# jlvdb/yet_another_wizz

Measured on AMD Instinct MI355X. Metric: candidate pairs/s, higher is better.
Workload: dtype f64

## Files before the change

### yet_another_wizz_amd/csrc/yawhip_band32.inc

```
namespace {

constexpr int B32_WAVES_PLAIN = 7;
constexpr int B32_WAVES_BIG = 6;
constexpr int B32_WAVES_W = 5;
constexpr int B32_WAVES_W1 = 5;
constexpr int B32_WAVES_LT = 1;
constexpr int band32_min_waves(int R, int CAP, bool WEIGHTED, int NE, bool UNI) {
    if (NE == 2 && UNI) {
        if (WEIGHTED) return R == 1 ? B32_WAVES_W1 : B32_WAVES_W;
        return CAP >= B32_CAP_BIG ? B32_WAVES_BIG : B32_WAVES_PLAIN;
    }
    return NE == 2 && !WEIGHTED ? B32_WAVES_LT : 1;
}

template <int R, int CAP, bool WEIGHTED, int NE, bool MERGED, bool UNI>
__global__ __launch_bounds__(64, band32_min_waves(R, CAP, WEIGHTED, NE, UNI))
void YAW_B32_NAME(const DevTab *__restrict__ tabs, const Item *__restrict__ items, int n_bins,
                  const double *__restrict__ t, const float *__restrict__ thr32,
                  const double *__restrict__ rwin_k, const float *__restrict__ ucap,
                  unsigned flush_mask, int swap,
                  unsigned long long *__restrict__ out_counts,
                  double *__restrict__ partials,
                  unsigned long long *__restrict__ counters, unsigned long long seg_cap) {
    static_assert(NE >= 2 && NE <= 4, "edges per bin");
// ... 6 lines not shown
    constexpr int NC = NE == 2 ? 1 : NE;
    constexpr int NF = NE - 1;
    constexpr int TW = thr32_width(NE);
    constexpr bool LANE_THR = MERGED && !UNI;
    extern __shared__ __attribute__((aligned(16))) unsigned char lds_dyn[];
    const int nkb = MERGED ? n_bins : 1;
    const int nslots = nkb * NF;
    unsigned char *p = lds_dyn;
    constexpr bool SLOT_TRIP = NE == 2 && !WEIGHTED && R == 2 && !LANE_THR;
    constexpr bool DOWN = SLOT_TRIP && CH == 1;
    constexpr int LEAD = DOWN ? 4 : 0;
    constexpr unsigned COLB = (CAP + 4 + LEAD) * 4;
    float *const stage_lead = reinterpret_cast<float *>(p);
    float *stage = stage_lead + LEAD; p += (size_t)3 * COLB;
    double *sw = reinterpret_cast<double *>(p); if (WEIGHTED) p += (size_t)(CAP + 4) * 8;
    HistT *hist = reinterpret_cast<HistT *>(p); p += (size_t)nslots * sizeof(HistT);
    p = reinterpret_cast<unsigned char *>(((size_t)p + 15) & ~(size_t)15);
    float *sthr = reinterpret_cast<float *>(p);
    const int lane = threadIdx.x;
    const unsigned a_stage = (unsigned)(size_t)(lds_byte *)reinterpret_cast<unsigned char *>(stage);
    const unsigned a_sw = (unsigned)(size_t)(lds_byte *)reinterpret_cast<unsigned char *>(sw);
    const unsigned a_hist = (unsigned)(size_t)(lds_byte *)reinterpret_cast<unsigned char *>(hist);

    const TicketMap tmap = ticket_map(counters, seg_cap);
    const unsigned long long n_kept = tmap.n_kept;
    for (int e = lane; e < nslots; e += 64) hist[e] = HistT(0);
    if constexpr (DOWN) {
        if (a_stage != 4u * LEAD) __builtin_trap();
        if (lane < LEAD) { stage_lead[lane] = PAD_COORD32; stage_lead[COLB / 4 + lane] = PAD_COORD32; stage_lead[2 * (COLB / 4) + lane] = PAD_COORD32; }
    }
    if (LANE_THR)
        for (int e = lane; e < n_bins * TW; e += 64) sthr[e] = thr32[e];
    unsigned round_no = 0;
    for (unsigned long long v = blockIdx.x;; v += gridDim.x) {
        if ((v >> 3) >= tmap.per_xcd) break;
        const unsigned long long ticket = tmap.ticket(v);
        if (ticket >= n_kept) continue;
        const Item it = items[ticket];
        const int o = item_orient(it), islot = item_slot(it);
        const DevTab cl = tabs[swap ? o : 3 + o], cs = tabs[swap ? 3 + o : o];
        const int kfix = MERGED ? 0 : islot % n_bins;
        const float rwin = (float)(rwin_k[kfix] * 1.000001 + 4e-7);

        int win = 0;
        int64_t win_off = 0;
        int64_t cb[CH];
        int cn[CH], co[CH];
        int nch = 0;
        auto next_round = [&]() {
            nch = 0;
            int used = 0;
#pragma unroll
            for (int c = 0; c < CH; ++c) {
                cb[c] = 0; cn[c] = 0; co[c] = 0;
                if (win < it.nwin && nch == c) {
                    const int64_t wb = win == 0 ? it.b0[0] : (win == 1 ? it.b0[1] : it.b0[2]);
                    const int64_t rem = (int64_t)(win == 0 ? it.nb[0] : (win == 1 ? it.nb[1] : it.nb[2])) - win_off;
                    if (rem + 1 <= (int64_t)(CAP - used)) {
                        cb[c] = wb + win_off; cn[c] = (int)rem; co[c] = used;
                        used += ((int)rem + 1 + 3) & ~3;
                        ++win; win_off = 0; ++nch;
                    } else if (c == 0) {
                        cb[c] = wb + win_off; cn[c] = CAP - 4; co[c] = 0;
                        used = CAP;
                        win_off += CAP - 4; ++nch;
                    }
// ... 6 lines not shown
                if (c < nch) {
                    const gf32p gx = cs.qx + cb[c], gy = cs.qy + cb[c], gz = cs.qz + cb[c];
                    const unsigned a_c = a_stage + ((unsigned)co[c] << 2);
#pragma unroll
                    for (int k = 0; k < (CAP + 255) / 256; ++k) {
                        const unsigned e = (unsigned)(k * 256 + 4 * lane);
                        if (e < (unsigned)cn[c]) {
                            __builtin_amdgcn_global_load_lds(gx + e, lds_ptr(a_c + k * 1024), 16, 0, 0);
                            __builtin_amdgcn_global_load_lds(gy + e, lds_ptr(a_c + COLB + k * 1024), 16, 0, 0);
                            __builtin_amdgcn_global_load_lds(gz + e, lds_ptr(a_c + 2 * COLB + k * 1024), 16, 0, 0);
                        }
                    }
                    if (WEIGHTED && cs.w) {
#pragma unroll
                        for (int k = 0; k < (CAP + 127) / 128; ++k) {
                            const unsigned e = (unsigned)(k * 128 + 2 * lane);
                            if (e < (unsigned)cn[c])
                                __builtin_amdgcn_global_load_lds(cs.w + cb[c] + e, lds_ptr(a_sw + ((unsigned)co[c] << 3) + k * 1024), 16, 0, 0);
                        }
                    }
                }
            }
        };
        __syncthreads();
        next_round();
        issue_round();
        f32x2 ax2[R / 2 > 0 ? R / 2 : 1], ay2[R / 2 > 0 ? R / 2 : 1], az2[R / 2 > 0 ? R / 2 : 1];
        float ax[R], ay[R], az[R];
        int kb[R];
        double aw_own[R];
        int lane_obj = lane;
        int n_own = (int)it.na - lane * R;
        n_own = n_own < 0 ? 0 : (n_own > R ? R : n_own);
#pragma unroll
        for (int r = 0; r < R; ++r) {
            const bool have = r < n_own;
            const unsigned ic = have ? (unsigned)(lane * R + r) : 0u;
            ax[r] = have ? (cl.qx + it.a0)[ic] : PAD_COORD32;
            ay[r] = have ? (cl.qy + it.a0)[ic] : PAD_COORD32;
            az[r] = have ? (cl.qz + it.a0)[ic] : PAD_COORD32;
            kb[r] = MERGED ? (have ? (cl.k + it.a0)[ic] : 0) : 0;
            if constexpr (WEIGHTED) aw_own[r] = (cl.w && have) ? (cl.w + it.a0)[ic] : 1.0;
        }
        float th[R][TW];
        {
            const float *row = LANE_THR ? nullptr : thr32 + (size_t)kfix * TW;
#pragma unroll
            for (int r = 0; r < R; ++r)
#pragma unroll
                for (int q = 0; q < TW; ++q) th[r][q] = LANE_THR ? sthr[kb[r] * TW + q] : row[q];
        }
        float klo, khi;
        {
            const int last_r = n_own > 0 ? n_own - 1 : 0;
            float u_first = cl.axis == 0 ? ax[0] : (cl.axis == 1 ? ay[0] : az[0]), u_last = u_first;
#pragma unroll
            for (int r = 1; r < R; ++r)
                if (r == last_r) u_last = cl.axis == 0 ? ax[r] : (cl.axis == 1 ? ay[r] : az[r]);
            klo = u_first - rwin;
            khi = u_last + rwin;
            const float cap_c = ucap[2 * kfix], cap_s = ucap[2 * kfix + 1];
            if (cap_s > 0.0f) {
                klo = cap_lo32(u_first, cap_c, cap_s);
                khi = cap_hi32(u_last, cap_c, cap_s);
            }
        }
        if constexpr (R >= 2) {
#pragma unroll
            for (int h = 0; h < R / 2; ++h) {
                ax2[h] = f32x2{ax[2 * h], ax[2 * h + 1]}; ay2[h] = f32x2{ay[2 * h], ay[2 * h + 1]}; az2[h] = f32x2{az[2 * h], az[2 * h + 1]};
            }
        }
        f32x2 nc2[R / 2 > 0 ? R / 2 : 1];
#pragma unroll
        for (int h = 0; h < R / 2; ++h) nc2[h] = f32x2{-th[2 * h][0], -th[2 * h + 1][0]};
        unsigned int cnt[R][NC];
        double acc[R][NC];
#pragma unroll
        for (int r = 0; r < R; ++r)
#pragma unroll
            for (int c = 0; c < NC; ++c) { cnt[r][c] = 0u; acc[r][c] = 0.0; }
        unsigned int nev = 0;
        constexpr bool HALF = R == 1 && CH == 1;
        const double pair_mult = HALF && (it.pad_ & 1) ? 2.0 : 1.0;
        auto flush_lanes = [&]() {
#pragma unroll
            for (int r = 0; r < R; ++r) {
#pragma unroll
                for (int f = 0; f < NF; ++f) {
                    const unsigned cell = a_hist + (unsigned)((kb[r] * NF + f) * (int)sizeof(HistT));
                    if constexpr (WEIGHTED) {
                        const double vsum = NE == 2 ? acc[r][0] : acc[r][f + 1] - acc[r][f];
                        const double aw = aw_own[r];
                        if (vsum != 0.0)
                            (void)__hip_atomic_fetch_add((__attribute__((address_space(3))) double *)(size_t)cell, HALF ? aw * vsum * pair_mult : aw * vsum,
                                                         __ATOMIC_RELAXED, __HIP_MEMORY_SCOPE_WORKGROUP);
                    } else {
                        const unsigned int c = (NE == 2 ? cnt[r][0] : cnt[r][f + 1] - cnt[r][f]) << (HALF ? (it.pad_ & 1) : 0);
                        if (c)
                            (void)__hip_atomic_fetch_add((__attribute__((address_space(3))) unsigned int *)(size_t)cell, c,
                                                         __ATOMIC_RELAXED, __HIP_MEMORY_SCOPE_WORKGROUP);
                    }
                }
#pragma unroll
                for (int c = 0; c < NC; ++c) { cnt[r][c] = 0u; acc[r][c] = 0.0; }
            }
        };
        auto flush_counts = [&]() {
            flush_lanes();
            __syncthreads();
            for (int idx = lane; idx < nslots; idx += 64) {
                const unsigned int c = (unsigned int)hist[idx];
                hist[idx] = HistT(0);
                if (c) atomicAdd(&out_counts[(int64_t)islot * nslots + idx], (unsigned long long)c);
            }
        };

        const bool single_window = it.nwin == 1 && it.nb[0] + 1 <= CAP;
        for (;; ++round_no) {
            asm volatile("s_waitcnt vmcnt(0)" ::: "memory");
            __syncthreads();
            if (lane < nch) {
                int at = co[0] + cn[0];
                if constexpr (CH > 1) at = lane == 0 ? at : (lane == 1 ? co[1] + cn[1] : co[CH - 1] + cn[CH - 1]);
                stage[at] = PAD_COORD32; stage[COLB / 4 + at] = PAD_COORD32; stage[2 * (COLB / 4) + at] = PAD_COORD32;
                if (WEIGHTED) sw[at] = 0.0;
                if constexpr (PAIRS) {
                    stage[at + 1] = PAD_COORD32; stage[COLB / 4 + at + 1] = PAD_COORD32; stage[2 * (COLB / 4) + at + 1] = PAD_COORD32;
                    if (WEIGHTED) sw[at + 1] = 0.0;
                }
            }
            if (WEIGHTED && !cs.w) {
#pragma unroll
                for (int c = 0; c < CH; ++c)
                    if (c < nch)
                        for (int e = lane; e < cn[c]; e += 64) sw[co[c] + e] = 1.0;
            }
            __syncthreads();
            unsigned a_key[CH], a_sent[CH], ql[CH], qh[CH];
            int n_max = 1;
#pragma unroll
            for (int c = 0; c < CH; ++c) {
                a_key[c] = a_stage + COLB * (unsigned)cl.axis + ((unsigned)co[c] << 2);
                a_sent[c] = a_key[c] + ((unsigned)cn[c] << 2);
                ql[c] = qh[c] = a_key[c] - 4u;
                n_max = cn[c] > n_max ? cn[c] : n_max;
            }
            for (unsigned step = 4u << (31 - __builtin_clz(n_max)); step >= 4u; step >>= 1) {
#pragma unroll
                for (int c = 0; c < CH; ++c) {
                    if (c < nch) {
                        const unsigned pl = ql[c] + step, ph = qh[c] + step;
                        const float kl = *(const __attribute__((address_space(3))) float *)(size_t)(pl < a_sent[c] ? pl : a_sent[c]);
                        const float kh = *(const __attribute__((address_space(3))) float *)(size_t)(ph < a_sent[c] ? ph : a_sent[c]);
                        ql[c] = kl < klo ? pl : ql[c];
                        qh[c] = kh <= khi ? ph : qh[c];
                    }
                }
            }
#pragma unroll
            for (int c = 0; c < CH; ++c) {
            if (c < nch) {
            const int n = cn[c];
            int lo = (int)((ql[c] + 4u - a_key[c]) >> 2), hi = (int)((qh[c] + 4u - a_key[c]) >> 2);
            if (n_own == 0) lo = hi = n;
            if constexpr (R == 1 && CH == 1) {
                if (it.pad_ & 1) {
                    const int own = n_own > 0 ? (int)((long long)(cl.pos3 + it.a0)[lane] - (long long)cb[c]) + 1 : n;
                    lo = own > lo ? own : lo;
                    lo = lo > hi ? hi : lo;
                }
            }
            int len = hi - lo;
            int top = hi - 1;
            unsigned stride = PAIRS ? 8u : 4u;
            nev += (unsigned int)(len * n_own);
            if (single_window) {
                const unsigned long long act = __builtin_amdgcn_ballot_w64(len > 0);
                const int first = act ? __builtin_ctzll(act) : 0, span = act ? 64 - __builtin_clzll(act) - first : 64;
                if (span <= 32) {
                    const int sh = span <= 8 ? 3 : (span <= 16 ? 2 : 1);
                    const bool idle = (lane >> sh) >= span;
                    const int src = idle ? first : first + (lane >> sh);
                    const int part = lane & ((1 << sh) - 1);
                    if constexpr (R >= 2) {
#pragma unroll
                        for (int h = 0; h < R / 2; ++h) {
                            ax2[h] = f32x2{__shfl(ax2[h].x, src, 64), __shfl(ax2[h].y, src, 64)};
                            ay2[h] = f32x2{__shfl(ay2[h].x, src, 64), __shfl(ay2[h].y, src, 64)};
                            az2[h] = f32x2{__shfl(az2[h].x, src, 64), __shfl(az2[h].y, src, 64)};
                        }
                    }
#pragma unroll
                    for (int r = 0; r < R; ++r) {
                        if constexpr (R < 2) { ax[r] = __shfl(ax[r], src, 64); ay[r] = __shfl(ay[r], src, 64); az[r] = __shfl(az[r], src, 64); }
                        if constexpr (MERGED) kb[r] = __shfl(kb[r], src, 64);
                        if constexpr (WEIGHTED) aw_own[r] = __shfl(aw_own[r], src, 64);
// ... 192 lines not shown
                    }
                }
            } else {
                auto eval_entry = [&](const unsigned a16) {
                    unsigned long long unc_mask[NS];
                    float s32[NS];
                    double ewi[NS];
                    if (__builtin_expect(classify_entry(a16, unc_mask, s32, ewi) != 0ull, 0)) settle_entry(a16, unc_mask, s32, ewi);
                };
                for (int s = 0; s < steps; ++s) {
                    eval_entry(cur < last ? cur : last);
                    cur += stride;
                }
            }
            }
            }
            if (!WEIGHTED && (round_no & flush_mask) == flush_mask) flush_counts();
            if (win >= it.nwin) break;
            __syncthreads();
            next_round();
            issue_round();
        }
        ++round_no;
        if constexpr (WEIGHTED) {
            flush_lanes();
            __syncthreads();
            for (int idx = lane; idx < nslots; idx += 64) {
                partials[(int64_t)it.pot * nslots + idx] = (double)hist[idx];
                hist[idx] = HistT(0);
            }
        } else {
            flush_counts();
        }
        nev = wave_sum_lane63(nev);
        if (lane == 63 && nev) atomicAdd(&counters[BAND_ENTRY_CTR(ticket & (EVAL_SLOTS - 1))], (unsigned long long)nev);
    }
}

}

namespace yawhip_detail {

hipError_t YAW_B32_LAUNCH(const CountLaunch &L, bool wgt, int32_t *variant) {
    const std::pair<int, int> stage{L.R, L.cap};
    const std::pair<bool, bool> rows{L.merged, L.uni};
    const dim3 band_grid(L.band_grid), wave(64);
    return pick<Bool<false>, Bool<true>>(wgt, [&](auto w) {
        return pick<Int<4>, Int<3>, Int<2>>(L.n_edges, [&](auto ne) {
            return pick<Rows<true, false>, Rows<true, true>, Rows<false, true>>(rows, [&](auto r) {
                return pick<Stage<4, B32_CAP_BIG>, Stage<2, B32_CAP_BIG>, Stage<2, B32_CAP>, Stage<1, B32_CAP>>(stage, [&](auto s) {
                    using S = decltype(s);
                    using M = decltype(r);
                    *variant = variant_code(YAW_B32_CH == 1 ? VF_BAND32_ONE : VF_BAND32, S::R, S::CAP, w, ne, M::MERGED, M::UNI);
                    return launch(YAW_B32_NAME<S::R, S::CAP, w, ne, M::MERGED, M::UNI>, band_grid, wave, L.lds, L.stream, L.d_tabs,
                                  L.d_items, L.n_bins, L.d_t, L.d_thr32, L.d_rwin, L.d_ucap, L.flush_mask, L.swap ? 1 : 0,
                                  L.d_counts, L.d_partials, L.d_ctr, L.seg_cap);
                });
            });
        });
    });
}

}
```

### yet_another_wizz_amd/csrc/yawhip_count.hip

```cpp

#include <hip/hip_runtime.h>

#include <algorithm>
#include <chrono>
#include <cmath>
#include <cstdint>
#include <cstdio>
#include <cstring>
#include <functional>
#include <memory>
#include <new>
#include <numeric>
#include <utility>
#include <vector>

#include "yawhip_count_kernels.h"

using namespace yawhip_detail;

namespace {
inline DevTab make_tab(const double *x, const double *y, const double *z, const double *w, const int32_t *k, const int64_t *off,
                       const int64_t *vbase, const int64_t *slo, const int64_t *tiles, const TileRec *tile_rec, const RunGrid *grid,
                       int axis, const float *q = nullptr, int64_t q_stride = 0, const int32_t *idx = nullptr) {
    return DevTab{(gf64p)x, (gf64p)y, (gf64p)z, (gf64p)w, (gi32p)k, (gi64p)off, (gi64p)vbase, (gi64p)slo, (gi64p)tiles,
                  tile_rec, grid, (gf32p)q, (gf32p)(q ? q + q_stride : nullptr), (gf32p)(q ? q + 2 * q_stride : nullptr), (gi32p)idx,
                  (gi32p)nullptr, axis, 0};
}

inline int64_t seg_len(const yawhip_catalog *c, int patch, int k) {
    const int kk = c->nb == 1 ? 0 : k;
    const int64_t i = (int64_t)patch * c->nb + kk;
    return c->h_off[i + 1] - c->h_off[i];
}

int32_t merge_variant(int32_t a, int32_t b) { return a == 0 || a == b ? b : (b == 0 ? a : YAWHIP_VARIANT_MIXED); }

std::vector<float> build_thr32(const double *t, int n_bins, int n_edges) {
    auto down = [](double v) { float f = (float)v; if ((double)f > v) f = nextafterf(f, -INFINITY); return f; };
    auto up = [](double v) { float f = (float)v; if ((double)f < v) f = nextafterf(f, INFINITY); return f; };
    auto guard = [](double te) { return BAND32_GUARD_SQRT * std::sqrt(te) + 5e-7 * te + 1e-12; };
    const int tw = thr32_width(n_edges);
    std::vector<float> out((size_t)n_bins * tw, 0.f);
    for (int k = 0; k < n_bins; ++k) {
        const double *tk = t + (size_t)k * n_edges;
        float *row = &out[(size_t)k * tw];
        if (n_edges == 2) {
            const double g0 = guard(tk[0]), g1 = guard(tk[1]);
            const float c = (float)(0.5 * (tk[0] + tk[1]));
            const double cd = (double)c;
            const double fold = 4e-7 * cd;
            const double h_in = (std::min(cd - (tk[0] + g0), (tk[1] - g1) - cd) - fold) * (1.0 - 1e-6);
            const double h_out = (std::max(cd - (tk[0] - g0), (tk[1] + g1) - cd) + fold) * (1.0 + 1e-6);
            row[0] = c;
            row[1] = h_in > 0.0 ? down(h_in) : 0.f;
            row[2] = up(std::max(h_out, 0.0));
            row[3] = 0.f;
        } else {
            for (int e = 0; e < n_edges; ++e) {
                const double g = guard(tk[e]);
// ... 458 lines not shown
              ((P.run_weighted && n_items * P.slab * (int64_t)sizeof(double) > ctx->slab_budget) || n_items >= (1ll << 31));
    return YAWHIP_OK;
}

int Planner::tables() {
    std::vector<float> dthr((size_t)3 * n_bins);
    auto round_down = [](double v) { float f = (float)v; if ((double)f > v) f = nextafterf(f, -4.0f); return f; };
    for (int k = 0; k < n_bins; ++k) {
        const double thi = t[(size_t)k * n_edges + n_edges - 1];
        float thr32 = ctx->debug_no_hits ? 2.0f : round_down(1.0 - 0.5 * thi - FILTER_GUARD);
        dthr[(size_t)3 * k] = thr32;
        dthr[(size_t)3 * k + 1] = 0.f;
        dthr[(size_t)3 * k + 2] = 0.f;
    }
    if (P.merged) rwin[0] = P.rwin_max;
    const bool trim = ctx->band_trim && c1->unit_norm && c2->unit_norm;
    std::vector<float> ucap((size_t)2 * n_bins);
    for (int k = 0; k < n_bins; ++k) {
        const double th = sep_angle(rwin[(size_t)k]);
        ucap[(size_t)2 * k] = trim ? (float)std::cos(th) : 1.0f;
        ucap[(size_t)2 * k + 1] = trim ? (float)std::sin(th) : 0.0f;
    }
    if (trim) {
        P.cap_c = std::cos(sep_angle(P.rwin_max));
        P.cap_s = std::sin(sep_angle(P.rwin_max));
    }
    DevTab h_tabs[6];
    memset(h_tabs, 0, sizeof h_tabs);
    if (P.strip_items) {
        for (int o = 0; o < 3; ++o) {
            if (!L1[o]) continue;
            const StripLayout &a = *L1[o], &b = *L2[o];
            h_tabs[o] = make_tab(a.x, a.y, a.z, a.w, P.merged ? a.k : nullptr, a.off, a.d_vbase, a.d_slo, a.d_tiles[tile_idx],
                                 a.d_tile_rec[tile_idx], a.d_grid, o, a.q, a.q_stride);
            h_tabs[3 + o] = make_tab(b.x, b.y, b.z, b.w, nullptr, b.off, b.d_vbase, b.d_slo, b.d_tiles[tile_idx],
                                     b.d_tile_rec[tile_idx], b.d_grid, o, b.q, b.q_stride);
            if (P.triple) {
                const StripLayout &st = P.swap ? b : a;
                DevTab &tb = h_tabs[P.swap ? 3 + o : o];
                tb = make_tab(st.x, st.y, st.z, st.w3, nullptr, st.off3, st.d_vbase, st.d_slo, st.d_tiles[tile_idx],
                              st.d_tile_rec[tile_idx], st.d_grid3, o, st.q3, st.q3_stride, st.idx3);
                if (half_ok) h_tabs[3 + o].pos3 = (gi32p)(const int32_t *)b.pos3;
            }
        }
    } else {
        h_tabs[0] = make_tab(c1->x, c1->y, c1->z, c1->w, nullptr, c1->off, nullptr, nullptr, nullptr, nullptr, nullptr, c1->axis);
        h_tabs[3] = make_tab(c2->x, c2->y, c2->z, c2->w, nullptr, c2->off, nullptr, nullptr, nullptr, nullptr, nullptr, c2->axis);
    }
    static_assert(sizeof(JobRec) == 8 * sizeof(int32_t), "JobRec is 32 bytes");
    const std::vector<float> thr32 = P.band32 ? build_thr32(t, n_bins, n_edges) : (P.band_fine ? fine32 : std::vector<float>());
    std::vector<int64_t> cprefix;
    if (P.run_weighted) {
        cprefix.assign((size_t)P.n_pslots + 1, 0);
        for (int64_t sl = 0; sl < P.n_pslots; ++sl)
            cprefix[(size_t)sl + 1] = cprefix[(size_t)sl] + (prefix[(size_t)sl + 1] - prefix[(size_t)sl] + REDUCE_CHUNK - 1) / REDUCE_CHUNK;
    }
    P.n_chunks = cprefix.empty() ? 0 : cprefix.back();
    const void *src[9] = {P.strip_items ? (const void *)job_recs.data() : (const void *)jobs, prefix.data(), t, dthr.data(),
                          rwin.data(), ucap.data(), thr32.data(), h_tabs, cprefix.data()};
    const size_t bytes[9] = {P.strip_items ? sizeof(JobRec) * (size_t)P.n_sjobs : sizeof(int32_t) * 2 * (size_t)n_jobs,
                             sizeof(int64_t) * ((size_t)P.n_pslots + 1), sizeof(double) * n_bins * n_edges, sizeof(float) * 3 * n_bins,
                             sizeof(double) * n_bins, sizeof(float) * 2 * n_bins, sizeof(float) * thr32.size(), sizeof h_tabs,
                             sizeof(int64_t) * cprefix.size()};
    size_t off[9], off_in = 0;
    for (int i = 0; i < 9; ++i) { off[i] = off_in; off_in = align16(off_in + bytes[i]); }
    std::vector<unsigned char> image(off_in, 0);
    for (int i = 0; i < 9; ++i)
        if (bytes[i]) memcpy(image.data() + off[i], src[i], bytes[i]);
    HIP_TRY(P.d_in.alloc(std::max<size_t>(off_in, 16)));
// ... 448 lines not shown
```

### yet_another_wizz_amd/csrc/yawhip_count_device.h

```cpp
#ifndef YAWHIP_COUNT_DEVICE_H
#define YAWHIP_COUNT_DEVICE_H
#include <hip/hip_runtime.h>

#include <algorithm>
#include <cstdint>
#include <type_traits>
#include <utility>

#include "yawhip_count_kernels.h"

using namespace yawhip_detail;

namespace {
constexpr double PAD_COORD = 4.0;

struct alignas(16) ObjF {
    float x, y, z, pad;
};

__device__ __forceinline__ double cap_lo64(double u, double c, double s) {
    const double ul = fmax(u - 1e-9, -1.0);
    return ul <= -c + 1e-12 ? -1.0 - 2e-9 : fma(ul, c, -sqrt(fmax(fma(-ul, ul, 1.0), 0.0)) * s) - 2e-9;
}
__device__ __forceinline__ double cap_hi64(double u, double c, double s) {
    const double uh = fmin(u + 1e-9, 1.0);
    return uh >= c - 1e-12 ? 1.0 + 2e-9 : fma(uh, c, sqrt(fmax(fma(-uh, uh, 1.0), 0.0)) * s) + 2e-9;
}
constexpr float CAP32_SHIFT = 1e-7f, CAP32_CLIP = 1.2e-7f, CAP32_MARGIN = 8e-7f;
__device__ __forceinline__ float cap_lo32(float u, float c, float s) {
    const float ul = fmaxf(u - CAP32_SHIFT, -1.0f);
    return ul <= -c + CAP32_CLIP ? -1.0f - CAP32_MARGIN : fmaf(ul, c, -sqrtf(fmaxf(fmaf(-ul, ul, 1.0f), 0.0f)) * s) - CAP32_MARGIN;
}
__device__ __forceinline__ float cap_hi32(float u, float c, float s) {
    const float uh = fminf(u + CAP32_SHIFT, 1.0f);
    return uh >= c - CAP32_CLIP ? 1.0f + CAP32_MARGIN : fmaf(uh, c, sqrtf(fmaxf(fmaf(-uh, uh, 1.0f), 0.0f)) * s) + CAP32_MARGIN;
}

constexpr int SLOT_MASK = 0x3fffffff;
__host__ __device__ inline int item_slot(const Item &it) { return it.slot & SLOT_MASK; }
__host__ __device__ inline int item_orient(const Item &it) { return (int)((unsigned)it.slot >> 30); }

typedef float f32x2 __attribute__((ext_vector_type(2)));
typedef float f32x4 __attribute__((ext_vector_type(4)));

__device__ __forceinline__ void stamp_start(unsigned long long *__restrict__ counters, int word) {
    if (blockIdx.x == 0 && threadIdx.x == 0) counters[word] = wall_clock64();
}

typedef __attribute__((address_space(3))) unsigned char lds_byte;
__device__ __forceinline__ __attribute__((address_space(3))) void *lds_ptr(unsigned addr) { return (__attribute__((address_space(3))) void *)(size_t)addr; }
__device__ __forceinline__ double lds_f64(unsigned addr) { return *(const __attribute__((address_space(3))) double *)(size_t)addr; }
__device__ __forceinline__ int lds_i32(unsigned addr) { return *(const __attribute__((address_space(3))) int *)(size_t)addr; }

__device__ __forceinline__ int wave_max_nonneg(int v) {
    v = max(v, __builtin_amdgcn_update_dpp(0, v, 0x111, 0xf, 0xf, false));
    v = max(v, __builtin_amdgcn_update_dpp(0, v, 0x112, 0xf, 0xf, false));
    v = max(v, __builtin_amdgcn_update_dpp(0, v, 0x114, 0xf, 0xf, false));
    v = max(v, __builtin_amdgcn_update_dpp(0, v, 0x118, 0xf, 0xf, false));
    v = max(v, __builtin_amdgcn_update_dpp(0, v, 0x142, 0xa, 0xf, false));
    v = max(v, __builtin_amdgcn_update_dpp(0, v, 0x143, 0xc, 0xf, false));
    return __builtin_amdgcn_readlane(v, 63);
}

__device__ __forceinline__ unsigned int wave_sum_lane63(unsigned int v) {
    v += (unsigned int)__builtin_amdgcn_update_dpp(0, (int)v, 0x111, 0xf, 0xf, false);
    v += (unsigned int)__builtin_amdgcn_update_dpp(0, (int)v, 0x112, 0xf, 0xf, false);
    v += (unsigned int)__builtin_amdgcn_update_dpp(0, (int)v, 0x114, 0xf, 0xf, false);
    v += (unsigned int)__builtin_amdgcn_update_dpp(0, (int)v, 0x118, 0xf, 0xf, false);
// ... 112 lines not shown
```

### yet_another_wizz_amd/csrc/yawhip_ingest.hip

```cpp

#include <hip/hip_runtime.h>

#include <algorithm>
#include <atomic>
#include <climits>
#include <cmath>
#include <cstdint>
#include <cstring>
#include <new>
#include <vector>

#include "yawhip_internal.h"

using namespace yawhip_detail;

namespace {

__global__ __launch_bounds__(256) void k_assign_patches(int64_t n, const double *__restrict__ x, const double *__restrict__ y,
                                                       const double *__restrict__ z, int n_centers,
                                                       const double *__restrict__ centers, int32_t *__restrict__ out) {
    extern __shared__ __attribute__((aligned(16))) unsigned char lds_raw[];
    double *c = reinterpret_cast<double *>(lds_raw);
    for (int e = threadIdx.x; e < 3 * n_centers; e += blockDim.x) c[e] = centers[e];
    __syncthreads();
// ... 54 lines not shown
}

__global__ __launch_bounds__(256) void k_segment_weight_sums(const double *__restrict__ w, const int64_t *__restrict__ off,
                                                            double *__restrict__ out) {
    __shared__ double part[256];
    const int64_t lo = off[blockIdx.x], hi = off[blockIdx.x + 1];
    double acc = 0.0;
    for (int64_t i = lo + threadIdx.x; i < hi; i += 256) acc += w[i];
    part[threadIdx.x] = acc;
    __syncthreads();
    for (int half = 128; half > 0; half >>= 1) {
        if ((int)threadIdx.x < half) part[threadIdx.x] += part[threadIdx.x + half];
        __syncthreads();
    }
    if (threadIdx.x == 0) out[blockIdx.x] = part[0];
}

__device__ __forceinline__ int segment_of(const int64_t *__restrict__ off, int n_seg, int64_t i) {
    int lo = 0, hi = n_seg;
    while (hi - lo > 1) {
        const int mid = (lo + hi) >> 1;
        if (off[mid] <= i) lo = mid; else hi = mid;
    }
    return lo;
}

__global__ void k_gather_bins(int64_t n, const uint32_t *__restrict__ perm, const int64_t *__restrict__ off, int64_t n_seg,
                              int n_bins, int32_t *__restrict__ bins) {
    const int64_t i = (int64_t)blockIdx.x * blockDim.x + threadIdx.x;
    if (i < n) bins[i] = segment_of(off, (int)n_seg, (int64_t)perm[i]) % n_bins;
}

__global__ void k_make_q(int64_t n, const double *__restrict__ x, const double *__restrict__ y, const double *__restrict__ z,
                         int64_t stride, float *__restrict__ q) {
    const int64_t i = (int64_t)blockIdx.x * blockDim.x + threadIdx.x;
    if (i >= n) return;
    q[i] = (float)x[i];
    q[stride + i] = (float)y[i];
    q[2 * stride + i] = (float)z[i];
}

__global__ void k_same_bin_neighbours(int64_t n, const int32_t *__restrict__ bins, unsigned long long *__restrict__ out) {
    const int64_t i = (int64_t)blockIdx.x * blockDim.x + threadIdx.x;
    const bool same = i + 1 < n && bins[i] == bins[i + 1];
    const unsigned long long m = __builtin_amdgcn_ballot_w64(same);
    if ((threadIdx.x & 63) == 0 && m) atomicAdd(out, (unsigned long long)__popcll(m));
}

__global__ void k_strip_index(int64_t n, const double *__restrict__ v, const double *__restrict__ u, const double *__restrict__ w,
                              double width, int lat, const int64_t *__restrict__ poff, int n_patches, int32_t *__restrict__ gidx,
                              int32_t *__restrict__ lohi) {
    const int64_t i = (int64_t)blockIdx.x * blockDim.x + threadIdx.x;
    const bool ok = i < n;
    int32_t g = 0;
    int p = -1;
    if (ok) {
        const double vi = v[i];
        if (width > 0.0)
            g = lat ? (int32_t)floor((atan2(vi, hypot(u[i], w[i])) + 1.5707963267948966) / width) : (int32_t)floor((vi + 1.0) / width);
        gidx[i] = g;
        p = segment_of(poff, n_patches, i);
    }
    const int p0 = __builtin_amdgcn_readfirstlane(p);
    if (__builtin_amdgcn_ballot_w64(p != p0) == 0ull) {
        if (p0 < 0) return;
        int32_t lo = g, hi = g;
        for (int off = 32; off > 0; off >>= 1) {
            lo = min(lo, __shfl_xor(lo, off, 64));
            hi = max(hi, __shfl_xor(hi, off, 64));
        }
        if ((threadIdx.x & 63) == 0) {
            atomicMin(&lohi[2 * p0], lo);
// ... 202 lines not shown
                       key_of(c->x, c->y, c->z, (saxis + 1) % 3), key_of(c->x, c->y, c->z, (saxis + 2) % 3), width, c->strip_grid && !seg ? 1 : 0, poff,
                       n_groups, gidx, lohi);
    e = hipMemcpyAsync(h_lohi.data(), lohi, (size_t)2 * n_groups * sizeof(int32_t), hipMemcpyDeviceToHost, ctx->stream);
    if (e == hipSuccess) e = hipStreamSynchronize(ctx->stream);
    if (e != hipSuccess) return bail(e, "strip index");
    std::vector<int64_t> vbase((size_t)n_groups + 1, 0), slo((size_t)n_groups, 0);
    for (int g = 0; g < n_groups; ++g) {
        const bool any = h_poff[(size_t)g + 1] > h_poff[(size_t)g];
        slo[(size_t)g] = any ? h_lohi[(size_t)2 * g] : 0;
        vbase[(size_t)g + 1] = vbase[(size_t)g] + (any ? (int64_t)h_lohi[(size_t)2 * g + 1] - h_lohi[(size_t)2 * g] + 1 : 0);
    }
    const int64_t n_runs = vbase[(size_t)n_groups];
    if (n_runs >= (1ll << 31)) return bail(hipErrorInvalidValue, "too many strip runs");
    int run_bits = 1;
    while ((1ll << run_bits) < n_runs) ++run_bits;
    e = L.d_vbase.alloc((size_t)(n_groups + 1));
    if (e == hipSuccess) e = L.d_slo.alloc((size_t)std::max(n_groups, 1));
    if (e == hipSuccess)
        e = hipMemcpyAsync(L.d_vbase, vbase.data(), (size_t)(n_groups + 1) * sizeof(int64_t), hipMemcpyHostToDevice, ctx->stream);
    if (e == hipSuccess)
        e = hipMemcpyAsync(L.d_slo, slo.data(), (size_t)n_groups * sizeof(int64_t), hipMemcpyHostToDevice, ctx->stream);
    if (e == hipSuccess) e = yawsort::sort_segments(ctx->sort_ws, ctx->stream, n, key_of(c->x, c->y, c->z, o), poff, n_groups, perm);
    if (e != hipSuccess) return bail(e, "group sort");
    hipLaunchKernelGGL(k_run_of, dim3(ngrid), dim3(256), 0, ctx->stream, n, perm, gidx, poff, n_groups, L.d_vbase, L.d_slo, run);
    e = yawsort::sort_runs(ctx->sort_ws, ctx->stream, n, run, perm, run_bits, perm2, run_sorted);
    if (e != hipSuccess) return bail(e, "run sort");
    e = L.x.alloc(n1, 16);
    if (e == hipSuccess) e = L.y.alloc(n1, 16);
    if (e == hipSuccess) e = L.z.alloc(n1, 16);
    if (e == hipSuccess && c->w) e = L.w.alloc(n1, 16);
    if (e == hipSuccess && want_bins) e = L.k.alloc(n1, 16);
    L.q_stride = (int64_t)((n1 + 3) & ~(size_t)3) + 8;
    if (e == hipSuccess) e = L.q.alloc((size_t)3 * L.q_stride);
    if (e == hipSuccess) e = L.off.alloc((size_t)(n_runs + 1));
    if (e == hipSuccess) e = L.d_grid.alloc((size_t)(n_runs + 1));
    if (e == hipSuccess) e = hipMemsetAsync(L.d_grid, 0, (size_t)(n_runs + 1) * sizeof(RunGrid), ctx->stream);
    if (e != hipSuccess) return bail(e, "strip layout");
    hipLaunchKernelGGL(k_gather_columns, dim3(ngrid), dim3(256), 0, ctx->stream, n, perm2, c->x, c->y, c->z, c->w, L.x, L.y, L.z, L.w);
    if (want_bins)
        hipLaunchKernelGGL(k_gather_bins, dim3(ngrid), dim3(256), 0, ctx->stream, n, perm2, c->off, nseg, c->nb, L.k);
    hipLaunchKernelGGL(k_make_q, dim3(ngrid), dim3(256), 0, ctx->stream, n, L.x, L.y, L.z, L.q_stride, L.q);
    hipLaunchKernelGGL(k_run_offsets, dim3((unsigned)((n_runs + 1 + 255) / 256)), dim3(256), 0, ctx->stream, run_sorted, n, n_runs,
                       L.off);
    if (n_runs > 0)
        hipLaunchKernelGGL(k_run_grid<double>, dim3((unsigned)((n_runs * (RUN_GRID + 1) + 255) / 256)), dim3(256), 0, ctx->stream, n_runs,
                           L.off, o == 0 ? L.x : (o == 1 ? L.y : L.z), L.d_grid);
    std::vector<int64_t> voff((size_t)n_runs + 1);
    e = hipMemcpyAsync(voff.data(), L.off, (size_t)(n_runs + 1) * sizeof(int64_t), hipMemcpyDeviceToHost, ctx->stream);
    unsigned long long h_same = 0;
    if (want_bins && n > 1) {
        unsigned long long *d_same = reinterpret_cast<unsigned long long *>(static_cast<uint32_t *>(run));
        if (e == hipSuccess) e = hipMemsetAsync(d_same, 0, sizeof(unsigned long long), ctx->stream);
        if (e == hipSuccess) {
            hipLaunchKernelGGL(k_same_bin_neighbours, dim3(ngrid), dim3(256), 0, ctx->stream, n, L.k, d_same);
            e = hipMemcpyAsync(&h_same, d_same, sizeof(unsigned long long), hipMemcpyDeviceToHost, ctx->stream);
        }
    }
    if (e == hipSuccess) e = hipStreamSynchronize(ctx->stream);
    if (e != hipSuccess) return bail(e, "run offsets");
    L.same_bin = n > 1 ? (double)h_same / (double)(n - 1) : 0.0;
    for (int64_t r = 0; r < n_runs; ++r)
        if (voff[(size_t)r + 1] - voff[(size_t)r] >= (1ll << 32)) return bail(hipErrorInvalidValue, "a strip run of 2^32 objects or more");
    for (int ri = 0; ri < 3; ++ri) {
        const int64_t tile = (int64_t)MWG << ri;
        L.h_tiles[ri].assign((size_t)n_runs + 1, 0);
        for (int64_t r = 0; r < n_runs; ++r)
            L.h_tiles[ri][(size_t)r + 1] = L.h_tiles[ri][(size_t)r] + (voff[(size_t)r + 1] - voff[(size_t)r] + tile - 1) / tile;
        {
            const int64_t n_tiles = L.h_tiles[ri][(size_t)n_runs];
            std::vector<TileRec> tile_rec((size_t)std::max<int64_t>(n_tiles, 1), TileRec{0, 0, 0, 0.0, 0.0});
            for (int64_t r = 0; r < n_runs; ++r)
                for (int64_t tl = L.h_tiles[ri][(size_t)r]; tl < L.h_tiles[ri][(size_t)r + 1]; ++tl) {
                    const int64_t a0 = voff[(size_t)r] + (tl - L.h_tiles[ri][(size_t)r]) * tile;
                    tile_rec[(size_t)tl] = TileRec{a0, (int32_t)std::min<int64_t>(tile, voff[(size_t)r + 1] - a0), (int32_t)r, 0.0, 0.0};
// ... 268 lines not shown
    return upload_catalogs(ctx, n, x, y, z, w, kappa ? kappa : &none, n_patches, n_bins_or_1, offsets, sort_axis, out_n, out_k);
}

int yawhip_catalog_segment_sums(const yawhip_catalog *cat, double *sums) {
    if (!cat || !sums) return fail(YAWHIP_ERR_INVALID, "yawhip_catalog_segment_sums: NULL argument");
    const int64_t nseg = (int64_t)cat->n_patches * cat->nb;
    if (!cat->w) {
        for (int64_t s = 0; s < nseg; ++s) sums[s] = (double)(cat->h_off[(size_t)s + 1] - cat->h_off[(size_t)s]);
        return YAWHIP_OK;
    }
    yawhip_ctx *ctx = cat->ctx;
    HIP_TRY(hipSetDevice(ctx->device));
    DevPtr<double> d_out;
    hipError_t e = d_out.alloc((size_t)nseg);
    if (e != hipSuccess) return fail(YAWHIP_ERR_OOM, "segment sums: %s", hipGetErrorString(e));
    hipLaunchKernelGGL(k_segment_weight_sums, dim3((unsigned)nseg), dim3(256), 0, ctx->stream, cat->w, cat->off, d_out);
    e = hipGetLastError();
    if (e == hipSuccess) e = hipMemcpyAsync(sums, d_out, (size_t)nseg * sizeof(double), hipMemcpyDeviceToHost, ctx->stream);
    if (e == hipSuccess) e = hipStreamSynchronize(ctx->stream);
    if (e != hipSuccess) return fail(YAWHIP_ERR_HIP, "segment sums failed: %s", hipGetErrorString(e));
    return YAWHIP_OK;
}

int yawhip_catalog_free(yawhip_catalog *c) {
    if (!c) return YAWHIP_OK;
    for (yawhip_catalog *rep : c->replicas) (void)yawhip_catalog_free(rep);
    c->replicas.clear();
    if (c->ctx) (void)hipSetDevice(c->ctx->device);
    if (c->ctx) {
        if (c->ctx->stream) (void)hipStreamSynchronize(c->ctx->stream);
        drop_plans(c->ctx, c);
    }
    delete c;
    return YAWHIP_OK;
}

int yawhip_catalog_device_bytes(const yawhip_catalog *cat, int64_t *bytes) {
    if (!cat || !bytes) return fail(YAWHIP_ERR_INVALID, "yawhip_catalog_device_bytes: NULL argument");
    *bytes = cat->device_bytes;
    return YAWHIP_OK;
}

int yawhip_assign_patches(yawhip_ctx *ctx, int64_t n, const double *x, const double *y, const double *z, int32_t n_centers,
                          const double *centers_xyz, int32_t *patch_out) {
    if (!ctx) return fail(YAWHIP_ERR_INVALID, "yawhip_assign_patches: ctx is NULL");
    if (n < 0 || n_centers <= 0 || !centers_xyz || (n > 0 && (!x || !y || !z || !patch_out)))
        return fail(YAWHIP_ERR_INVALID, "yawhip_assign_patches: bad sizes or NULL arrays");
    if ((size_t)n_centers * 3 * sizeof(double) > (size_t)ctx->lds_limit)
        return fail(YAWHIP_ERR_INVALID, "too many centres (%d) for the LDS table", n_centers);
    if (n == 0) return YAWHIP_OK;
    HIP_TRY(hipSetDevice(ctx->device));
    DevPtr<double> dx, dc;
    DevPtr<int32_t> dout;
    hipError_t e = dx.alloc((size_t)3 * n);
    if (e == hipSuccess) e = dc.alloc((size_t)3 * n_centers);
    if (e == hipSuccess) e = dout.alloc((size_t)n);
    if (e == hipSuccess) e = hipMemcpyAsync(dx, x, (size_t)n * sizeof(double), hipMemcpyHostToDevice, ctx->stream);
    if (e == hipSuccess) e = hipMemcpyAsync(dx + n, y, (size_t)n * sizeof(double), hipMemcpyHostToDevice, ctx->stream);
    if (e == hipSuccess) e = hipMemcpyAsync(dx + 2 * n, z, (size_t)n * sizeof(double), hipMemcpyHostToDevice, ctx->stream);
    if (e == hipSuccess)
        e = hipMemcpyAsync(dc, centers_xyz, (size_t)3 * n_centers * sizeof(double), hipMemcpyHostToDevice, ctx->stream);
    if (e == hipSuccess) {
        const size_t lds = (size_t)3 * n_centers * sizeof(double);
        if (lds > 64 * 1024)
            e = hipFuncSetAttribute(reinterpret_cast<const void *>(k_assign_patches), hipFuncAttributeMaxDynamicSharedMemorySize, (int)lds);
        if (e == hipSuccess) {
// ... 13 lines not shown
```

### yet_another_wizz_amd/csrc/yawhip_internal.h

```cpp
#ifndef YAWHIP_INTERNAL_H
#define YAWHIP_INTERNAL_H
#include <hip/hip_runtime.h>

#include <chrono>
#include <cstddef>
#include <cstdint>
#include <cstdio>
#include <cstdlib>
#include <cstring>
#include <functional>
#include <string>
#include <utility>
#include <vector>

#include "yawhip.h"
#include "yawhip_devmem.h"
#include "yawhip_healpix.h"
#include "yawhip_sort.h"

#pragma GCC visibility push(hidden)

namespace yawhip_detail {
struct Trace {
    bool on = getenv("YAWHIP_TRACE") != nullptr;
// ... 31 lines not shown
#define HIP_TRY(expr)                                                                              \
    do {                                                                                           \
        hipError_t e_ = (expr);                                                                    \
        if (e_ != hipSuccess)                                                                      \
            return fail(e_ == hipErrorOutOfMemory ? YAWHIP_ERR_OOM : YAWHIP_ERR_HIP, "%s failed: %s (%s:%d)", \
                        #expr, hipGetErrorString(e_), __FILE__, __LINE__);                         \
    } while (0)

struct CatView {
    const double *x, *y, *z, *w;
    const int64_t *off;
    int nb;
    const double *key;
    int axis;
};

constexpr int MAX_WIN = 3;
struct alignas(16) Item {
    int64_t a0;
    int32_t na;
    int32_t slot;
    int32_t pot;
    int32_t nwin;
    int64_t b0[MAX_WIN];
    int32_t nb[MAX_WIN];
    int32_t pad_;
};
static_assert(sizeof(Item) == 64, "Item layout");

typedef const __attribute__((address_space(1))) double *gf64p;
typedef const __attribute__((address_space(1))) int32_t *gi32p;
typedef const __attribute__((address_space(1))) int64_t *gi64p;
typedef const __attribute__((address_space(1))) float *gf32p;
struct DevTab {
    gf64p x, y, z, w;
    gi32p k;
    gi64p off;
    gi64p vbase, slo, tiles;
    const struct TileRec *tile_rec;
    const struct RunGrid *grid;
    gf32p qx, qy, qz;
    gi32p idx;
    gi32p pos3;
    int32_t axis;
    int32_t pad_;
};
__device__ __forceinline__ gf64p tab_key(const DevTab &t) { return t.axis == 0 ? t.x : (t.axis == 1 ? t.y : t.z); }

struct alignas(16) TileRec {
    int64_t a0;
    int32_t na;
    int32_t run;
    double klo, khi;
};
static_assert(sizeof(TileRec) == 32, "TileRec is read as two 16-byte words");
struct JobRec {
    int64_t t_lo;
    int64_t k_off;
    int64_t vbase1;
    int32_t n_strips1;
    int32_t o;
};
constexpr int RUN_GRID = 64;
struct alignas(16) RunGrid {
    int64_t b0;
    double first, last;
    double inv;
    uint32_t n;
    uint32_t g[RUN_GRID + 1];
};
static_assert(sizeof(RunGrid) == 304 && offsetof(RunGrid, n) == 32, "RunGrid: a 36-byte head in front of g[]");
constexpr int64_t RUN_GRID_ACCOUNTED = 8 + 4 * (RUN_GRID + 2), TILE_REC_ACCOUNTED = 16;
__device__ __forceinline__ int run_cell(double key, double first, double inv) {
    const double f = (key - first) * inv;
// ... 87 lines not shown
    const double *t = nullptr;
    std::vector<int32_t> own_jobs;
    std::vector<double> own_t;

    CallKey() = default;
    CallKey(const yawhip_ctx *ctx, const CountArgs &a, bool want_counts, bool want_sums, bool for_work,
            int32_t n_dev = 0);
    CallKey(CallKey &&) = default;
    CallKey &operator=(CallKey &&) = default;
    CallKey(const CallKey &) = delete;
    CallKey &operator=(const CallKey &) = delete;

    void keep() {
        own_jobs.assign(jobs, jobs + 2 * (size_t)n_jobs);
        own_t.assign(t, t + (size_t)n_bins * n_edges);
        jobs = own_jobs.data();
        t = own_t.data();
    }
    bool operator==(const CallKey &o) const {
        return hash == o.hash && c1_uid == o.c1_uid && c2_uid == o.c2_uid && opt_gen == o.opt_gen && n_jobs == o.n_jobs &&
               n_bins == o.n_bins && n_edges == o.n_edges && kernel == o.kernel && n_dev == o.n_dev && want_counts == o.want_counts &&
               want_sums == o.want_sums && for_work == o.for_work &&
               memcmp(jobs, o.jobs, sizeof(int32_t) * 2 * (size_t)n_jobs) == 0 &&
               memcmp(t, o.t, sizeof(double) * (size_t)n_bins * n_edges) == 0;
    }
};

struct StripLayout {
    bool built = false;
    DevPtr<double> x, y, z, w;
    DevPtr<int32_t> k;
    DevPtr<float> q;
    int64_t q_stride = 0;
    DevPtr<int64_t> off;
    std::vector<int64_t> h_off;
    std::vector<int64_t> h_vbase;
    std::vector<int64_t> h_slo;
    std::vector<int64_t> h_tiles[3];
    DevPtr<int64_t> d_vbase, d_slo, d_tiles[3];
    DevPtr<TileRec> d_tile_rec[3];
    DevPtr<RunGrid> d_grid;
    bool triples = false;
    DevPtr<float> q3;
    int64_t q3_stride = 0;
    DevPtr<double> w3;
    DevPtr<int32_t> idx3;
    DevPtr<int32_t> pos3;
    DevPtr<int64_t> off3;
    DevPtr<RunGrid> d_grid3;
    int64_t n_groups = 0;
    int64_t device_bytes = 0;
    double obj_run = 0.0;
    double same_bin = 0.0;
    void release_triples() {
        q3.release(); w3.release(); idx3.release(); pos3.release(); off3.release(); d_grid3.release();
        triples = false;
    }
    void release() { *this = StripLayout{}; }
};

}

struct yawhip_ctx : yawhip_detail::CallBufs {
    int device = 0;
    hipStream_t stream = nullptr;
    int tile_r = 0;
// ... 123 lines not shown
```

Before: 35060000 billion.

## Pack per-object coords and bin into 16-byte records; rework band search and entry counting

Adds an interleaved float4 image (x,y,z,bin) per strip layout so each lane loads its owned objects with a single 16-byte load instead of four separate strided loads. The binary search over staged keys changes from a clamped power-of-two step search to a halving-count search with a final fix-up compare, which drops the per-step sentinel clamp. Entry-counter atomics are batched across tickets and only flushed when a lane counter nears overflow, and the cap bound computations use the raw hardware sqrt. The cost is extra device memory and ingest work for the new image, plus a debug entry point to check it.

```diff
diff --git a/yet_another_wizz_amd/csrc/yawhip_band32.inc b/yet_another_wizz_amd/csrc/yawhip_band32.inc
--- a/yet_another_wizz_amd/csrc/yawhip_band32.inc
+++ b/yet_another_wizz_amd/csrc/yawhip_band32.inc
@@ -62,6 +62,12 @@
     if (LANE_THR)
         for (int e = lane; e < n_bins * TW; e += 64) sthr[e] = thr32[e];
     unsigned round_no = 0;
+    unsigned int nev = 0;
+    auto send_entries = [&](unsigned int lane_sum) {
+        const unsigned int lo16 = wave_sum_lane63(lane_sum & 0xffffu), hi16 = wave_sum_lane63(lane_sum >> 16);
+        const unsigned long long sum = (unsigned long long)lo16 + ((unsigned long long)hi16 << 16);
+        if (lane == 63 && sum) atomicAdd(&counters[BAND_ENTRY_CTR(blockIdx.x & (EVAL_SLOTS - 1))], sum);
+    };
     for (unsigned long long v = blockIdx.x;; v += gridDim.x) {
         if ((v >> 3) >= tmap.per_xcd) break;
         const unsigned long long ticket = tmap.ticket(v);
@@ -134,14 +140,20 @@
         int lane_obj = lane;
         int n_own = (int)it.na - lane * R;
         n_own = n_own < 0 ? 0 : (n_own > R ? R : n_own);
+        lane_words rec[R];
+        {
+            const glanep lane_q = cl.q4 + it.a0 + lane * R;
+#pragma unroll
+            for (int r = 0; r < R; ++r) rec[r] = lane_q[r];
+        }
 #pragma unroll
         for (int r = 0; r < R; ++r) {
             const bool have = r < n_own;
             const unsigned ic = have ? (unsigned)(lane * R + r) : 0u;
-            ax[r] = have ? (cl.qx + it.a0)[ic] : PAD_COORD32;
-            ay[r] = have ? (cl.qy + it.a0)[ic] : PAD_COORD32;
-            az[r] = have ? (cl.qz + it.a0)[ic] : PAD_COORD32;
-            kb[r] = MERGED ? (have ? (cl.k + it.a0)[ic] : 0) : 0;
+            ax[r] = have ? rec[r].x : PAD_COORD32;
+            ay[r] = have ? rec[r].y : PAD_COORD32;
+            az[r] = have ? rec[r].z : PAD_COORD32;
+            kb[r] = MERGED ? (have ? __float_as_int(rec[r].w) : 0) : 0;
             if constexpr (WEIGHTED) aw_own[r] = (cl.w && have) ? (cl.w + it.a0)[ic] : 1.0;
         }
         float th[R][TW];
@@ -182,7 +194,6 @@
         for (int r = 0; r < R; ++r)
 #pragma unroll
             for (int c = 0; c < NC; ++c) { cnt[r][c] = 0u; acc[r][c] = 0.0; }
-        unsigned int nev = 0;
         constexpr bool HALF = R == 1 && CH == 1;
         const double pair_mult = HALF && (it.pad_ & 1) ? 2.0 : 1.0;
         auto flush_lanes = [&]() {
@@ -239,24 +250,26 @@
                         for (int e = lane; e < cn[c]; e += 64) sw[co[c] + e] = 1.0;
             }
             __syncthreads();
-            unsigned a_key[CH], a_sent[CH], ql[CH], qh[CH];
-            int n_max = 1;
+            unsigned a_key[CH], ql[CH], qh[CH];
+            int left[CH], left_max = 0;
 #pragma unroll
             for (int c = 0; c < CH; ++c) {
                 a_key[c] = a_stage + COLB * (unsigned)cl.axis + ((unsigned)co[c] << 2);
-                a_sent[c] = a_key[c] + ((unsigned)cn[c] << 2);
                 ql[c] = qh[c] = a_key[c] - 4u;
-                n_max = cn[c] > n_max ? cn[c] : n_max;
-            }
-            for (unsigned step = 4u << (31 - __builtin_clz(n_max)); step >= 4u; step >>= 1) {
+                left[c] = cn[c];
+                left_max = cn[c] > left_max ? cn[c] : left_max;
+            }
+            for (; left_max > 1; left_max -= left_max >> 1) {
 #pragma unroll
                 for (int c = 0; c < CH; ++c) {
-                    if (c < nch) {
-                        const unsigned pl = ql[c] + step, ph = qh[c] + step;
-                        const float kl = *(const __attribute__((address_space(3))) float *)(size_t)(pl < a_sent[c] ? pl : a_sent[c]);
-                        const float kh = *(const __attribute__((address_space(3))) float *)(size_t)(ph < a_sent[c] ? ph : a_sent[c]);
+                    if (c < nch && (CH == 1 || left[c] > 1)) {
+                        const unsigned half4 = (unsigned)(left[c] >> 1) << 2;
+                        const unsigned pl = ql[c] + half4, ph = qh[c] + half4;
+                        const float kl = *(const __attribute__((address_space(3))) float *)(size_t)pl;
+                        const float kh = *(const __attribute__((address_space(3))) float *)(size_t)ph;
                         ql[c] = kl < klo ? pl : ql[c];
                         qh[c] = kh <= khi ? ph : qh[c];
+                        left[c] -= left[c] >> 1;
                     }
                 }
             }
@@ -265,6 +278,8 @@
             if (c < nch) {
             const int n = cn[c];
             int lo = (int)((ql[c] + 4u - a_key[c]) >> 2), hi = (int)((qh[c] + 4u - a_key[c]) >> 2);
+            lo += *(const __attribute__((address_space(3))) float *)(size_t)(ql[c] + 4u) < klo ? 1 : 0;
+            hi += *(const __attribute__((address_space(3))) float *)(size_t)(qh[c] + 4u) <= khi ? 1 : 0;
             if (n_own == 0) lo = hi = n;
             if constexpr (R == 1 && CH == 1) {
                 if (it.pad_ & 1) {
@@ -523,9 +538,9 @@
         } else {
             flush_counts();
         }
-        nev = wave_sum_lane63(nev);
-        if (lane == 63 && nev) atomicAdd(&counters[BAND_ENTRY_CTR(ticket & (EVAL_SLOTS - 1))], (unsigned long long)nev);
+        if (__builtin_amdgcn_ballot_w64((int)nev < 0)) { send_entries(nev); nev = 0; }
     }
+    send_entries(nev);
 }
 
 }
diff --git a/yet_another_wizz_amd/csrc/yawhip_count.hip b/yet_another_wizz_amd/csrc/yawhip_count.hip
--- a/yet_another_wizz_amd/csrc/yawhip_count.hip
+++ b/yet_another_wizz_amd/csrc/yawhip_count.hip
@@ -21,10 +21,11 @@
 namespace {
 inline DevTab make_tab(const double *x, const double *y, const double *z, const double *w, const int32_t *k, const int64_t *off,
                        const int64_t *vbase, const int64_t *slo, const int64_t *tiles, const TileRec *tile_rec, const RunGrid *grid,
-                       int axis, const float *q = nullptr, int64_t q_stride = 0, const int32_t *idx = nullptr) {
+                       int axis, const float *q = nullptr, int64_t q_stride = 0, const int32_t *idx = nullptr,
+                       const LaneObj *q4 = nullptr) {
     return DevTab{(gf64p)x, (gf64p)y, (gf64p)z, (gf64p)w, (gi32p)k, (gi64p)off, (gi64p)vbase, (gi64p)slo, (gi64p)tiles,
-                  tile_rec, grid, (gf32p)q, (gf32p)(q ? q + q_stride : nullptr), (gf32p)(q ? q + 2 * q_stride : nullptr), (gi32p)idx,
-                  (gi32p)nullptr, axis, 0};
+                  tile_rec, grid, (gf32p)q, (gf32p)(q ? q + q_stride : nullptr), (gf32p)(q ? q + 2 * q_stride : nullptr), (glanep)q4,
+                  (gi32p)idx, (gi32p)nullptr, axis, 0};
 }
 
 inline int64_t seg_len(const yawhip_catalog *c, int patch, int k) {
@@ -549,9 +550,9 @@
             if (!L1[o]) continue;
             const StripLayout &a = *L1[o], &b = *L2[o];
             h_tabs[o] = make_tab(a.x, a.y, a.z, a.w, P.merged ? a.k : nullptr, a.off, a.d_vbase, a.d_slo, a.d_tiles[tile_idx],
-                                 a.d_tile_rec[tile_idx], a.d_grid, o, a.q, a.q_stride);
+                                 a.d_tile_rec[tile_idx], a.d_grid, o, a.q, a.q_stride, nullptr, a.q4);
             h_tabs[3 + o] = make_tab(b.x, b.y, b.z, b.w, nullptr, b.off, b.d_vbase, b.d_slo, b.d_tiles[tile_idx],
-                                     b.d_tile_rec[tile_idx], b.d_grid, o, b.q, b.q_stride);
+                                     b.d_tile_rec[tile_idx], b.d_grid, o, b.q, b.q_stride, nullptr, b.q4);
             if (P.triple) {
                 const StripLayout &st = P.swap ? b : a;
                 DevTab &tb = h_tabs[P.swap ? 3 + o : o];
diff --git a/yet_another_wizz_amd/csrc/yawhip_count_device.h b/yet_another_wizz_amd/csrc/yawhip_count_device.h
--- a/yet_another_wizz_amd/csrc/yawhip_count_device.h
+++ b/yet_another_wizz_amd/csrc/yawhip_count_device.h
@@ -27,13 +27,17 @@
     return uh >= c - 1e-12 ? 1.0 + 2e-9 : fma(uh, c, sqrt(fmax(fma(-uh, uh, 1.0), 0.0)) * s) + 2e-9;
 }
 constexpr float CAP32_SHIFT = 1e-7f, CAP32_CLIP = 1.2e-7f, CAP32_MARGIN = 8e-7f;
+__device__ __forceinline__ float cap32_clipped(float bound) {
+    asm volatile("" : "+v"(bound));
+    return bound;
+}
 __device__ __forceinline__ float cap_lo32(float u, float c, float s) {
-    const float ul = fmaxf(u - CAP32_SHIFT, -1.0f);
-    return ul <= -c + CAP32_CLIP ? -1.0f - CAP32_MARGIN : fmaf(ul, c, -sqrtf(fmaxf(fmaf(-ul, ul, 1.0f), 0.0f)) * s) - CAP32_MARGIN;
+    const float ul = fmaxf(u - CAP32_SHIFT, -1.0f), clipped = cap32_clipped(-1.0f - CAP32_MARGIN);
+    return ul <= -c + CAP32_CLIP ? clipped : fmaf(ul, c, -__builtin_amdgcn_sqrtf(fmaxf(fmaf(-ul, ul, 1.0f), 0.0f)) * s) - CAP32_MARGIN;
 }
 __device__ __forceinline__ float cap_hi32(float u, float c, float s) {
-    const float uh = fminf(u + CAP32_SHIFT, 1.0f);
-    return uh >= c - CAP32_CLIP ? 1.0f + CAP32_MARGIN : fmaf(uh, c, sqrtf(fmaxf(fmaf(-uh, uh, 1.0f), 0.0f)) * s) + CAP32_MARGIN;
+    const float uh = fminf(u + CAP32_SHIFT, 1.0f), clipped = cap32_clipped(1.0f + CAP32_MARGIN);
+    return uh >= c - CAP32_CLIP ? clipped : fmaf(uh, c, __builtin_amdgcn_sqrtf(fmaxf(fmaf(-uh, uh, 1.0f), 0.0f)) * s) + CAP32_MARGIN;
 }
 
 constexpr int SLOT_MASK = 0x3fffffff;
diff --git a/yet_another_wizz_amd/csrc/yawhip_ingest.hip b/yet_another_wizz_amd/csrc/yawhip_ingest.hip
--- a/yet_another_wizz_amd/csrc/yawhip_ingest.hip
+++ b/yet_another_wizz_amd/csrc/yawhip_ingest.hip
@@ -110,12 +110,18 @@
 }
 
 __global__ void k_make_q(int64_t n, const double *__restrict__ x, const double *__restrict__ y, const double *__restrict__ z,
-                         int64_t stride, float *__restrict__ q) {
-    const int64_t i = (int64_t)blockIdx.x * blockDim.x + threadIdx.x;
-    if (i >= n) return;
-    q[i] = (float)x[i];
-    q[stride + i] = (float)y[i];
-    q[2 * stride + i] = (float)z[i];
+                         const int32_t *__restrict__ bins, int64_t stride, float *__restrict__ q, LaneObj *__restrict__ q4) {
+    const int64_t i = (int64_t)blockIdx.x * blockDim.x + threadIdx.x;
+    if (i >= n + LANE_IMAGE_PAD) return;
+    if (i >= n) {
+        q4[i] = LaneObj{0.0f, 0.0f, 0.0f, 0};
+        return;
+    }
+    const float fx = (float)x[i], fy = (float)y[i], fz = (float)z[i];
+    q[i] = fx;
+    q[stride + i] = fy;
+    q[2 * stride + i] = fz;
+    q4[i] = LaneObj{fx, fy, fz, bins ? bins[i] : 0};
 }
 
 __global__ void k_same_bin_neighbours(int64_t n, const int32_t *__restrict__ bins, unsigned long long *__restrict__ out) {
@@ -384,6 +390,7 @@
     if (e == hipSuccess && want_bins) e = L.k.alloc(n1, 16);
     L.q_stride = (int64_t)((n1 + 3) & ~(size_t)3) + 8;
     if (e == hipSuccess) e = L.q.alloc((size_t)3 * L.q_stride);
+    if (e == hipSuccess) e = L.q4.alloc((size_t)(n + LANE_IMAGE_PAD));
     if (e == hipSuccess) e = L.off.alloc((size_t)(n_runs + 1));
     if (e == hipSuccess) e = L.d_grid.alloc((size_t)(n_runs + 1));
     if (e == hipSuccess) e = hipMemsetAsync(L.d_grid, 0, (size_t)(n_runs + 1) * sizeof(RunGrid), ctx->stream);
@@ -391,7 +398,8 @@
     hipLaunchKernelGGL(k_gather_columns, dim3(ngrid), dim3(256), 0, ctx->stream, n, perm2, c->x, c->y, c->z, c->w, L.x, L.y, L.z, L.w);
     if (want_bins)
         hipLaunchKernelGGL(k_gather_bins, dim3(ngrid), dim3(256), 0, ctx->stream, n, perm2, c->off, nseg, c->nb, L.k);
-    hipLaunchKernelGGL(k_make_q, dim3(ngrid), dim3(256), 0, ctx->stream, n, L.x, L.y, L.z, L.q_stride, L.q);
+    hipLaunchKernelGGL(k_make_q, dim3((unsigned)((n + LANE_IMAGE_PAD + 255) / 256)), dim3(256), 0, ctx->stream, n, L.x, L.y, L.z,
+                       want_bins ? (const int32_t *)L.k : nullptr, L.q_stride, L.q, L.q4);
     hipLaunchKernelGGL(k_run_offsets, dim3((unsigned)((n_runs + 1 + 255) / 256)), dim3(256), 0, ctx->stream, run_sorted, n, n_runs,
                        L.off);
     if (n_runs > 0)
@@ -726,6 +734,30 @@
         drop_plans(c->ctx, c);
     }
     delete c;
+    return YAWHIP_OK;
+}
+
+int yawhip_debug_lane_image(yawhip_ctx *ctx, yawhip_catalog *cat, int32_t o, int32_t seg, int64_t *n_checked, int64_t *n_differing) {
+    if (!ctx || !cat || !n_checked || !n_differing || o < 0 || o > 2) return fail(YAWHIP_ERR_INVALID, "yawhip_debug_lane_image: bad argument");
+    if (cat->strip_width <= 0.0 || (seg && cat->nb <= 1)) return fail(YAWHIP_ERR_INVALID, "yawhip_debug_lane_image: no such layout");
+    if (const int rc = build_strip_layout(ctx, cat, o, seg != 0)) return rc;
+    const StripLayout &L = seg ? cat->seg[o] : cat->strips[o];
+    const int64_t n = cat->n;
+    std::vector<LaneObj> rec((size_t)(n + LANE_IMAGE_PAD));
+    std::vector<float> q((size_t)3 * L.q_stride);
+    std::vector<int32_t> bins((size_t)n, 0);
+    HIP_TRY(hipSetDevice(ctx->device));
+    HIP_TRY(hipMemcpy(rec.data(), L.q4, rec.size() * sizeof(LaneObj), hipMemcpyDeviceToHost));
+    HIP_TRY(hipMemcpy(q.data(), L.q, q.size() * sizeof(float), hipMemcpyDeviceToHost));
+    if (L.k && n > 0) HIP_TRY(hipMemcpy(bins.data(), L.k, (size_t)n * sizeof(int32_t), hipMemcpyDeviceToHost));
+    int64_t bad = 0;
+    for (int64_t i = 0; i < n + LANE_IMAGE_PAD; ++i) {
+        const LaneObj want = i < n ? LaneObj{q[(size_t)i], q[(size_t)(L.q_stride + i)], q[(size_t)(2 * L.q_stride + i)], bins[(size_t)i]}
+                                   : LaneObj{0.0f, 0.0f, 0.0f, 0};
+        bad += memcmp(&rec[(size_t)i], &want, sizeof(LaneObj)) != 0;
+    }
+    *n_checked = n;
+    *n_differing = bad;
     return YAWHIP_OK;
 }
 
diff --git a/yet_another_wizz_amd/csrc/yawhip_internal.h b/yet_another_wizz_amd/csrc/yawhip_internal.h
--- a/yet_another_wizz_amd/csrc/yawhip_internal.h
+++ b/yet_another_wizz_amd/csrc/yawhip_internal.h
@@ -87,6 +87,14 @@
 typedef const __attribute__((address_space(1))) int32_t *gi32p;
 typedef const __attribute__((address_space(1))) int64_t *gi64p;
 typedef const __attribute__((address_space(1))) float *gf32p;
+struct alignas(16) LaneObj {
+    float x, y, z;
+    int32_t bin;
+};
+static_assert(sizeof(LaneObj) == 16, "LaneObj is read with one 16-byte load");
+constexpr int64_t LANE_IMAGE_PAD = 256;
+typedef float lane_words __attribute__((ext_vector_type(4)));
+typedef const __attribute__((address_space(1))) lane_words *glanep;
 struct DevTab {
     gf64p x, y, z, w;
     gi32p k;
@@ -95,6 +103,7 @@
     const struct TileRec *tile_rec;
     const struct RunGrid *grid;
     gf32p qx, qy, qz;
+    glanep q4;
     gi32p idx;
     gi32p pos3;
     int32_t axis;
@@ -248,6 +257,7 @@
     DevPtr<int32_t> k;
     DevPtr<float> q;
     int64_t q_stride = 0;
+    DevPtr<LaneObj> q4;
     DevPtr<int64_t> off;
     std::vector<int64_t> h_off;
     std::vector<int64_t> h_vbase;
```

Result: faster. 35770000 billion, median of 6 (+2.0%).
